# sephiroce/srf

Measured on AMD Instinct MI355X. Metric: acoustic frames/sec through SRF (123-d fbank, 3-iter DR) at 1/2/4/8 MI355X, higher is better.
Workload: dtype fp32; 1 GPU; wsj_c4: SRF L=6 PH=CH=16 DIM=32 LPAD=RPAD=2 DR iter=3, train step (fwd+bwd+allreduce+Adam); utterances_per_gpu=28, frames_per_utterance=800, global_batch=28, parallelism=dp1, launch=hipgraph (fwd+CTC+bwd)

## Files before the change

### srf_amd/csrc/route_dr.hip

```cpp
#include <algorithm>
#include <cmath>
#include <type_traits>

#include "srf_common.h"
#include "route_fwd32.h"
#include "../../include/srf.h"
#include "../../include/srf_prof.h"

namespace {

constexpr float kSquashEps = 1e-7f;

thread_local hipEvent_t* t_ev_start = nullptr;
thread_local hipEvent_t* t_ev_stop = nullptr;
thread_local int t_ev_n = 0;
constexpr int MODE_FWD = 0;
constexpr int MODE_BWD = 1;

using srf::DrGeom;

template <int KS>
__device__ __forceinline__ void load_vec(const float* __restrict__ p, float (&v)[KS]) {
  if constexpr (KS % 4 == 0) {
#pragma unroll
// ... 557 lines not shown
  const int lane = threadIdx.x & 63, wv = threadIdx.x >> 6;
  const int fl = lane & 15, g = lane >> 4;
  const int chunk = blockIdx.x % n_chunks;
  const int rest = blockIdx.x / n_chunks;
  const int wgrp = rest % n_wgroups;
  const int ft = rest / n_wgroups;
  const int f = ft * 16 + fl;
  const FrameLoc loc = frame_loc(f, F, T);
  const int tbase = __builtin_amdgcn_readfirstlane((wgrp * NW + wv) * TW);
  const int n0 = chunk * n_per, nn = min(N, n0 + n_per) - n0;
  const int Wn = in_n / N;
  const int ncap = Wn * nn;
  const int Jeff = J - (mask_first ? 1 : 0);
  const int SROW = gu_row_stride(n_per, DIN);
  const int nslots = 15 + Wn;
  float* gw_acc = gacc + (size_t)wv * nslots_max * SROW;
  for (int k = threadIdx.x; k < NW * nslots_max * SROW; k += blockDim.x) gacc[k] = 0.f;
  __syncthreads();

  float vcr[RV][TW][4], gsr[R][TW][4];
  float c0[TW];
#pragma unroll
  for (int t = 0; t < TW; ++t) {
    const int j = tile_j<DIN>(tbase + t, g);
    c0[t] = (j < J && !(mask_first && j == 0)) ? 1.f / (float)Jeff : 0.f;
#pragma unroll
    for (int r = 0; r < R; ++r) {
      if (r > 0) load_rows(saved + (size_t)(2 * (r - 1) + 1) * FJD, f, loc.valid, JD, tbase + t, g, vcr[r - 1][t]);
      load_rows(gs + (size_t)r * FJD, f, loc.valid, JD, tbase + t, g, gsr[r][t]);
    }
  }
  const int Fs = srf::fwd32_frame_stride(F);
  const uint32_t cblk_b = (uint32_t)in_n * JP * Fs * 4;
  const auto rs_w = __builtin_amdgcn_make_buffer_rsrc(const_cast<float*>(WT), 0, (int)((size_t)in_n * NT * 16 * DIN * 4),
                                                       0x00020000);
  const auto rs_c = __builtin_amdgcn_make_buffer_rsrc(const_cast<float*>(cst), 0, (int)(cblk_b * RV), 0x00020000);
  const auto rs_g = __builtin_amdgcn_make_buffer_rsrc(const_cast<float*>(glst), 0, (int)(cblk_b * RV), 0x00020000);
  uint32_t wo[NCT][TW], co[TW];
#pragma unroll
  for (int t = 0; t < TW; ++t) {
    const int tc = min(tbase + t, NT - 1);
#pragma unroll
    for (int ct = 0; ct < NCT; ++ct)
      wo[ct][t] = (uint32_t)(((tc * 4 + g) * DIN + min(ct * 16 + fl, DIN - 1)) * 4) * 4;
    co[t] = (uint32_t)(min(tile_j<DIN>(tbase + t, g), J - 1) * Fs + (loc.valid ? f : 0)) * 4;
  }
  constexpr int NB = 3;
  f4 wt_b[NB][NCT][TW];
  float c_b[NB][RV][TW], g_b[NB][RV][TW];
  auto fetch = [&](auto slot, int i) {
    constexpr int sl = decltype(slot)::value;
    const uint32_t sw = (uint32_t)i * NT * 16 * DIN * 4;
    const uint32_t sc = (uint32_t)i * JP * Fs * 4;
#pragma unroll
    for (int ct = 0; ct < NCT; ++ct)
#pragma unroll
      for (int t = 0; t < TW; ++t)
        wt_b[sl][ct][t] = __builtin_bit_cast(f4, __builtin_amdgcn_raw_buffer_load_b128(rs_w, wo[ct][t], sw, 0));
#pragma unroll
    for (int r = 0; r < RV; ++r)
#pragma unroll
      for (int t = 0; t < TW; ++t) {
        c_b[sl][r][t] = __builtin_bit_cast(float, __builtin_amdgcn_raw_buffer_load_b32(rs_c, co[t], sc + r * cblk_b, 0));
        g_b[sl][r][t] = __builtin_bit_cast(float, __builtin_amdgcn_raw_buffer_load_b32(rs_g, co[t], sc + r * cblk_b, 0));
      }
  };
  int w = 0, nl = 0, wf = 0, nf = 0;
  auto advance = [&](int& ww, int& nn_) {
    if (++nn_ == nn) nn_ = 0, ++ww;
  };
  auto compute = [&](auto slot) {
    constexpr int sl = decltype(slot)::value;
    const int i = w * N + n0 + nl;
    float ga[TW][4];
#pragma unroll
    for (int t = 0; t < TW; ++t)
#pragma unroll
      for (int h = 0; h < 2; ++h) {
        f2 a = c0[t] * f2{gsr[0][t][2 * h], gsr[0][t][2 * h + 1]};
#pragma unroll
        for (int r = 0; r < RV; ++r) {
          a = c_b[sl][r][t] * f2{gsr[r + 1][t][2 * h], gsr[r + 1][t][2 * h + 1]} + a;
          a = g_b[sl][r][t] * f2{vcr[r][t][2 * h], vcr[r][t][2 * h + 1]} + a;
        }
        ga[t][2 * h] = a.x;
        ga[t][2 * h + 1] = a.y;
      }
    f4 gx[NCT];
#pragma unroll
    for (int ct = 0; ct < NCT; ++ct) {
      gx[ct] = f4{0.f, 0.f, 0.f, 0.f};
#pragma unroll
      for (int t = 0; t < TW; ++t)
#pragma unroll
        for (int q = 0; q < 4; ++q) gx[ct] = mfma16x16x4(wt_b[sl][ct][t][q], ga[t][q], gx[ct]);
    }
    const int ts = loc.t + w - lpad;
    if (loc.valid && ts >= 0 && ts < T) {
      const int n = i - w * N;
#pragma unroll
      for (int ct = 0; ct < NCT; ++ct) {
        if (ct * 16 + 4 * g >= DIN) continue;
        float* a = gw_acc + (fl + w) * SROW + gu_acc_col<DIN>(fl + w, (n - n0) * DIN + ct * 16 + 4 * g);
        st4(a, ld4(a) + gx[ct]);
      }
    }
    advance(w, nl);
  };
  using S0 = std::integral_constant<int, 0>;
  using S1 = std::integral_constant<int, 1>;
  using S2 = std::integral_constant<int, 2>;
  const int i_last = (Wn - 1) * N + n0 + nn - 1;
  auto next_i = [&]() {
    const int i = min(wf * N + n0 + nf, i_last);
    advance(wf, nf);
    return i;
  };
#define SRF_GUX_FETCH(SL) \
  fetch(SL{}, next_i());  \
  __builtin_amdgcn_sched_barrier(0);
  if (ncap > 0) {
    SRF_GUX_FETCH(S0)
    SRF_GUX_FETCH(S1)
  }
  for (int k = 0; k < ncap; k += NB) {
    SRF_GUX_FETCH(S2)
    compute(S0{});
    if (k + 1 >= ncap) break;
    SRF_GUX_FETCH(S0)
    compute(S1{});
    if (k + 2 >= ncap) break;
    SRF_GUX_FETCH(S1)
    compute(S2{});
  }
#undef SRF_GUX_FETCH
  __syncthreads();
  const int f0 = ft * 16 - lpad;
  const int row = nn * DIN;
  for (int k = threadIdx.x; k < nslots * row; k += blockDim.x) {
    const int slot = k / row, rem = k - slot * row;
    const int fo = f0 + slot;
    float v = 0.f;
    const int pos = gu_acc_col<DIN>(slot, rem);
    for (int q = 0; q < NW; ++q) v += gacc[((size_t)q * nslots_max + slot) * SROW + pos];
    if (fo >= 0 && fo < F && v != 0.f) atomicAdd(g_emb + ((size_t)fo * N + n0) * DIN + rem, v);
  }
}

#ifndef SRF_GUX16_XCD
#define SRF_GUX16_XCD 1
#endif
#ifndef SRF_GW16S_XCD
#define SRF_GW16S_XCD 1
#endif
typedef _Float16 h8 __attribute__((ext_vector_type(8)));
typedef float f16v __attribute__((ext_vector_type(16)));
typedef _Float16 h2 __attribute__((ext_vector_type(2)));
constexpr int kGux16NW = 4;
constexpr int kGux16Occ = 2;

__device__ __forceinline__ f16v mfma32h(const h8& a, const h8& b, const f16v& c) {
  return __builtin_amdgcn_mfma_f32_32x32x16_f16(a, b, c, 0, 0, 0);
}

__device__ __forceinline__ void split8h(const f2 (&a)[4], h8& hi, h8& lo) {
#pragma unroll
  for (int v = 0; v < 4; ++v) {
    const f2 hf = __builtin_bit_cast(f2, __builtin_bit_cast(u2, a[v]) & 0xFFFFE000u);
    const h2 ph = __builtin_convertvector(hf, h2), pl = __builtin_convertvector(a[v] - hf, h2);
    hi[2 * v] = ph[0];
    hi[2 * v + 1] = ph[1];
    lo[2 * v] = pl[0];
    lo[2 * v + 1] = pl[1];
  }
}

template <int R>
__global__ __launch_bounds__(64 * kGux16NW, kGux16Occ) void route_gux16_kernel(
    const float* __restrict__ WT, const float* __restrict__ hdr, int F, int T, int N, int lpad, int in_n, int J,
    int mask_first, int n_wgroups, int n_chunks, int n_per, const float* __restrict__ saved,
    const float* __restrict__ gs, float* __restrict__ g_emb, const float* __restrict__ cst,
    const float* __restrict__ glst, int JP, float* __restrict__ gumax, int jgpw) {
  static_assert(R >= 2, "stored couplings exist for iters >= 2");
  constexpr int DIN = 32, RV = R - 1, NW = kGux16NW;
  extern __shared__ __attribute__((aligned(16))) float gacc[];
  const int JD = J * DIN;
  const int NT = JD / 16;
  const size_t FJD = (size_t)F * JD;
  const int lane = threadIdx.x & 63, wv = threadIdx.x >> 6;
  const int fl = lane & 31, h = lane >> 5;
#if SRF_GUX16_XCD
  const int n_ft = (F + 31) / 32, n_tasks = n_ft * n_wgroups * n_chunks;
  const int task = (int)(blockIdx.x & 7) * (int)(gridDim.x >> 3) + (int)(blockIdx.x >> 3);
  if (task >= n_tasks) return;
  const int chunk = task % n_chunks;
  const int rest = task / n_chunks;
  const int ft = rest % n_ft;
  const int wgrp = rest / n_ft;
#else
  const int chunk = blockIdx.x % n_chunks;
  const int rest = blockIdx.x / n_chunks;
  const int wgrp = rest % n_wgroups;
  const int ft = rest / n_wgroups;
#endif
  const int f = ft * 32 + fl;
  const FrameLoc loc = frame_loc(f, F, T);
  const int fv = loc.valid ? f : 0;
  const int n0 = chunk * n_per, nn = min(N, n0 + n_per) - n0;
  const int Wn = in_n / N;
  const int ncap = Wn * nn;
  const int Jeff = J - (mask_first ? 1 : 0);
  const int SROW = n_per * DIN + 4;
  const int nslots = 31 + Wn;
  float* slab = gacc + (size_t)wv * nslots * SROW;
  for (int k = threadIdx.x; k < NW * nslots * SROW / 4; k += blockDim.x) st4(gacc + 4 * k, f4{0.f, 0.f, 0.f, 0.f});
  __syncthreads();
  float gmax = 0.f;
  for (int jg = 0; jg < jgpw; ++jg) {
  const int jw = (wgrp * jgpw + jg) * NW + wv;
  const bool wave_on = jw < J;
  const int j = __builtin_amdgcn_readfirstlane(min(jw, J - 1));

  const float c0 = (wave_on && !(mask_first && j == 0)) ? 1.f / (float)Jeff : 0.f;
  float gsr[R][16], vcr[RV][16];
  {
    const bool ok = loc.valid && wave_on;
    auto rows = [&](const float* base, float (&o)[16]) {
      const float* p = base + (size_t)fv * JD + j * DIN + 8 * h;
#pragma unroll
      for (int ks = 0; ks < 2; ++ks)
#pragma unroll
        for (int q = 0; q < 2; ++q) {
          const f4 a = ld4(p + 16 * ks + 4 * q);
          o[8 * ks + 4 * q] = ok ? a.x : 0.f;
          o[8 * ks + 4 * q + 1] = ok ? a.y : 0.f;
          o[8 * ks + 4 * q + 2] = ok ? a.z : 0.f;
          o[8 * ks + 4 * q + 3] = ok ? a.w : 0.f;
        }
    };
#pragma unroll
    for (int r = 0; r < R; ++r) {
      rows(gs + (size_t)r * FJD, gsr[r]);
      if (r > 0) rows(saved + (size_t)(2 * (r - 1) + 1) * FJD, vcr[r - 1]);
    }
  }
  float gm[R], vm[RV];
  {
    auto rowmax = [&](const float (&o)[16]) {
      float m = 0.f;
#pragma unroll
      for (int k = 0; k < 16; k += 2) m = fmaxf(m, fmaxf(fabsf(o[k]), fabsf(o[k + 1])));
      float ma, mb;
      xpair32(m, ma, mb);
      return fmaxf(ma, mb);
    };
#pragma unroll
    for (int r = 0; r < R; ++r) {
      gm[r] = rowmax(gsr[r]);
      if (r > 0) vm[r - 1] = rowmax(vcr[r - 1]);
    }
    gm[0] *= c0;
  }
  const int aw = (int)hdr[1];
  const int Fs = srf::fwd32_frame_stride(F);
  const uint32_t cblk_b = (uint32_t)in_n * JP * Fs * 4;
  const uint32_t wplane = (uint32_t)in_n * NT * 16 * DIN * 2;
  const auto rs_w = __builtin_amdgcn_make_buffer_rsrc(const_cast<float*>(WT), 0, (int)(2 * wplane), 0x00020000);
  const auto rs_c = __builtin_amdgcn_make_buffer_rsrc(const_cast<float*>(cst), 0, (int)(cblk_b * RV), 0x00020000);
  const auto rs_g = __builtin_amdgcn_make_buffer_rsrc(const_cast<float*>(glst), 0, (int)(cblk_b * RV), 0x00020000);
  uint32_t wo[2][2];
#pragma unroll
  for (int ks = 0; ks < 2; ++ks)
#pragma unroll
    for (int p = 0; p < 2; ++p) wo[ks][p] = (uint32_t)((((2 * j + ks) * 2 + h) * DIN + fl) * 16) + p * wplane;
  const uint32_t co = (uint32_t)(j * Fs + fv) * 4;
  constexpr int NB = 3;
  h8 wt_b[NB][2][2];
  float c_b[NB][RV], g_b[NB][RV];
  auto fetch = [&](auto slot, int i) {
    constexpr int sl = decltype(slot)::value;
    const uint32_t swo = (uint32_t)i * NT * 16 * DIN * 2;
    const uint32_t sc = (uint32_t)i * JP * Fs * 4;
#pragma unroll
    for (int ks = 0; ks < 2; ++ks)
#pragma unroll
      for (int p = 0; p < 2; ++p)
        wt_b[sl][ks][p] = __builtin_bit_cast(h8, __builtin_amdgcn_raw_buffer_load_b128(rs_w, wo[ks][p], swo, 0));
#pragma unroll
    for (int r = 0; r < RV; ++r) {
      c_b[sl][r] = __builtin_bit_cast(float, __builtin_amdgcn_raw_buffer_load_b32(rs_c, co, sc + r * cblk_b, 0));
      g_b[sl][r] = __builtin_bit_cast(float, __builtin_amdgcn_raw_buffer_load_b32(rs_g, co, sc + r * cblk_b, 0));
    }
  };
  int w = 0, nl = 0, wf = 0, nf = 0;
  auto advance = [&](int& ww, int& nn_) {
    if (++nn_ == nn) nn_ = 0, ++ww;
  };
  auto compute = [&](auto slot) {
    constexpr int sl = decltype(slot)::value;
    float mh = gm[0];
#pragma unroll
    for (int r = 0; r < RV; ++r) mh = fmaf(fabsf(g_b[sl][r]), vm[r], fmaf(fabsf(c_b[sl][r]), gm[r + 1], mh));
    gmax = fmaxf(gmax, mh);
    const int eg = srf_split_exp(mh);
    const float sg = srf_exp2i(eg);
    const float s0 = c0 * sg;
// ... 382 lines not shown
  constexpr int SF = CAP * PC;
  constexpr int SFL = CAP * PCL;
  constexpr int NQ = (SF / 4 + 255) / 256;
  __shared__ __attribute__((aligned(16))) float stg[2][SFL];
  const int JD = J * D;
  const int NT = (JD + 15) / 16;
  const size_t FJD = (size_t)F * JD;
  const int Fs = srf::fwd32_frame_stride(F);
  const size_t cblk = (size_t)in_n * JP * Fs;
  const int lane = threadIdx.x & 63, wv = threadIdx.x >> 6;
  const int l16 = lane & 15, kk = lane >> 4;
  int L = blockIdx.x;
  const int s = L % S;
  L /= S;
  const int rtg = L % n_rt;
  const int cc = L / n_rt;
  const int tg = rtg * 4 + wv;
  const int row = min(tg * 16 + l16, JD - 1);
  const bool rvalid = tg < NT && tg * 16 + l16 < JD;
  const int j = row / D;
  const int jg0 = (rtg * 64) / D;
  const int jl = min(j - jg0, JW - 1);
  const int Jeff = J - (mask_first ? 1 : 0);
  const float c0 = (rvalid && j < J && !(mask_first && j == 0)) ? 1.f / (float)Jeff : 0.f;
  const int i0 = cc * CAP, ncap = min(in_n, i0 + CAP) - i0;
  const int NFT = Fp >> 4;
  const int ft0 = s * ft_per, ft1 = min(NFT, ft0 + ft_per);

  const float* src[NQ];
  int dst[NQ];
#pragma unroll
  for (int q = 0; q < NQ; ++q) {
    const int idx = min(q * 256 + (int)threadIdx.x, SF / 4 - 1);
    const int k = idx / (PC / 4), rem = idx - k * (PC / 4);
    const int i = i0 + min(k, ncap - 1);
    if (rem < CG / 4) {
      const int fq = rem & 3, jw = (rem >> 2) % JW, cg = (rem >> 2) / JW;
      const int jj = min(jg0 + jw, JP - 1);
      src[q] = ((cg & 1) ? glst : cst) + (size_t)(cg >> 1) * cblk + ((size_t)i * JP + jj) * Fs + 4 * fq;
      dst[q] = k * PCL + rem * 4;
    } else {
      const int x = rem - CG / 4;
      src[q] = xT + ((size_t)i * D + (x >> 2)) * Fp + 4 * (x & 3);
      const int e = x >> 2;
      dst[q] = k * PCL + CG + e * 16 + 4 * ((x & 3) ^ ((e >> 1) & 3));
    }
  }
  f4 sv[NQ];
  auto stage_load = [&](int ft) {
#pragma unroll
    for (int q = 0; q < NQ; ++q) sv[q] = ld4(src[q] + ft * 16);
  };
  auto stage_store = [&](int buf) {
#pragma unroll
    for (int q = 0; q < NQ; ++q) {
      const int idx = q * 256 + threadIdx.x;
      if ((SF / 4) % 256 == 0 || idx < SF / 4) st4(&stg[buf][dst[q]], sv[q]);
    }
  };
  const uint32_t nrec = (uint32_t)(FJD * 4);
  __amdgpu_buffer_rsrc_t rs_g[R], rs_v[RV];
#pragma unroll
  for (int r = 0; r < R; ++r) {
    rs_g[r] = __builtin_amdgcn_make_buffer_rsrc(const_cast<float*>(gs + (size_t)r * FJD), 0, (int)nrec, 0x00020000);
    if (r > 0)
      rs_v[r - 1] = __builtin_amdgcn_make_buffer_rsrc(const_cast<float*>(saved + (size_t)(2 * (r - 1) + 1) * FJD), 0,
                                                      (int)nrec, 0x00020000);
  }
  const uint32_t vo0 = (uint32_t)((4 * kk) * JD + row) * 4;
  float g0[4], gr[RV][4], vr[RV][4];
  float n0[4], nr[RV][4], nvr[RV][4];
  auto vec_load = [&](int ft) {
#pragma unroll
    for (int v = 0; v < 4; ++v) {
      const uint32_t o = vo0 + (uint32_t)((ft * 16 + v) * JD) * 4;
      n0[v] = __builtin_bit_cast(float, __builtin_amdgcn_raw_buffer_load_b32(rs_g[0], o, 0, 0));
#pragma unroll
      for (int r = 0; r < RV; ++r) {
        nr[r][v] = __builtin_bit_cast(float, __builtin_amdgcn_raw_buffer_load_b32(rs_g[r + 1], o, 0, 0));
        nvr[r][v] = __builtin_bit_cast(float, __builtin_amdgcn_raw_buffer_load_b32(rs_v[r], o, 0, 0));
      }
    }
  };

  f4 acc[CAP][NCT];
  float gb[CAP];
#pragma unroll
  for (int k = 0; k < CAP; ++k) {
    gb[k] = 0.f;
#pragma unroll
    for (int ct = 0; ct < NCT; ++ct) acc[k][ct] = f4{0.f, 0.f, 0.f, 0.f};
  }
  if (ft0 < ft1) {
    stage_load(ft0);
    vec_load(ft0);
    stage_store(0);
    if (ft0 + 1 < ft1) stage_load(ft0 + 1);
  }
  for (int ft = ft0; ft < ft1; ++ft) {
    const int buf = (ft - ft0) & 1;
#pragma unroll
    for (int v = 0; v < 4; ++v) {
      g0[v] = n0[v];
#pragma unroll
      for (int r = 0; r < RV; ++r) gr[r][v] = nr[r][v], vr[r][v] = nvr[r][v];
    }
    __syncthreads();
    if (ft + 1 < ft1) {
      stage_store(buf ^ 1);
      if (ft + 2 < ft1) stage_load(ft + 2);
    }
    vec_load(ft + 1 < ft1 ? ft + 1 : ft);
    const float* sb = stg[buf];
#pragma unroll
    for (int k = 0; k < CAP; ++k) {
      const float* ck = sb + k * PCL;
      float gu[4];
#pragma unroll
      for (int v = 0; v < 4; ++v) gu[v] = c0 * g0[v];
#pragma unroll
      for (int r = 0; r < RV; ++r) {
        const f4 c = ld4(ck + ((r * 2 + 0) * JW + jl) * 16 + 4 * kk);
        const f4 gl = ld4(ck + ((r * 2 + 1) * JW + jl) * 16 + 4 * kk);
#pragma unroll
        for (int v = 0; v < 4; ++v) gu[v] += c[v] * gr[r][v] + gl[v] * vr[r][v];
      }
      gb[k] += (gu[0] + gu[1]) + (gu[2] + gu[3]);
#pragma unroll
      for (int ct = 0; ct < NCT; ++ct) {
        const int e = min(ct * 16 + l16, D - 1);
        const f4 xa = ld4(ck + CG + e * 16 + 4 * (kk ^ ((e >> 1) & 3)));
#pragma unroll
        for (int v = 0; v < 4; ++v) acc[k][ct] = mfma16x16x4(xa[v], gu[v], acc[k][ct]);
      }
    }
  }
  float* gw = gwp + (size_t)s * pstride;
  float* gbo = gbp + (size_t)s * pstride;
#pragma unroll
  for (int k = 0; k < CAP; ++k) {
    if (k >= ncap) continue;
    const int i = i0 + k;
    const float t = xor32_sum(xor16_sum(gb[k]));
    if (rvalid) {
      if (kk == 0) gbo[(size_t)i * JD + row] = t;
#pragma unroll
      for (int ct = 0; ct < NCT; ++ct)
        if (ct * 16 + 4 * kk < D) st4(gw + ((size_t)i * JD + row) * D + ct * 16 + 4 * kk, acc[k][ct]);
    }
  }
}

constexpr int kGw16Cap = 4;
template <int R, int CAP>
__global__ __launch_bounds__(256, 2) void route_gw16s_kernel(
    const _Float16* __restrict__ x16, const float* __restrict__ hdr, const float* __restrict__ gumax,
    const float* __restrict__ saved, const float* __restrict__ gs, const float* __restrict__ cst,
    const float* __restrict__ glst, int F, int Fp, int in_n, int J, int mask_first, int JP, int n_rt, int S,
    int ft_per, float* __restrict__ gwp, float* __restrict__ gbp, size_t pstride) {
  static_assert(R >= 2 && R <= 3, "stored couplings exist for iters >= 2; registers hold R <= 3");
  constexpr int D = 32, RV = R - 1;
  constexpr int CG = RV * 2 * 4 * 16;
  constexpr int PQ = CG / 4 + 128;
  constexpr int PCB = CG * 4 + 2 * D * 16 * 2;
  constexpr int NQ = (CAP * PQ + 255) / 256;
  __shared__ __attribute__((aligned(16))) unsigned char stg[2][CAP * PCB];
  const int JD = J * D;
  const size_t FJD = (size_t)F * JD;
  const int Fs = srf::fwd32_frame_stride(F);
  const size_t cblk = (size_t)in_n * JP * Fs;
  const int lane = threadIdx.x & 63, wv = threadIdx.x >> 6;
  const int n = lane & 31, h = lane >> 5;
#if SRF_GW16S_XCD
  const int n_cc = (in_n + CAP - 1) / CAP, n_tasks = n_cc * n_rt * S;
  const int task = (int)(blockIdx.x & 7) * (int)(gridDim.x >> 3) + (int)(blockIdx.x >> 3);
  if (task >= n_tasks) return;
  const int cc = task % n_cc;
  const int rtg = (task / n_cc) % n_rt;
  const int s = task / n_cc / n_rt;
#else
  int b = blockIdx.x;
  const int s = b % S;
  b /= S;
  const int rtg = b % n_rt;
  const int cc = b / n_rt;
#endif
  const int jw = rtg * 4 + wv;
  const bool wave_on = jw < J;
  const int j = min(jw, J - 1);
  const int row = j * D + n;
  const int Jeff = J - (mask_first ? 1 : 0);
  const float c0 = (wave_on && !(mask_first && j == 0)) ? 1.f / (float)Jeff : 0.f;
  const int i0 = cc * CAP, ncap = min(in_n, i0 + CAP) - i0;
  const int NFT = Fp >> 4;
  const int ft0 = s * ft_per, ft1 = min(NFT, ft0 + ft_per);
  const int bx = (int)hdr[2];
  const int eg = srf_split_exp(*gumax);
  const float sg = srf_exp2i(eg);

  constexpr int NCPL = CAP * CG / 4;
  const char* src[NQ];
  int dst[NQ];
  bool cpl[NQ];
#pragma unroll
  for (int q = 0; q < NQ; ++q) {
    const int idx = min(q * 256 + (int)threadIdx.x, CAP * PQ - 1);
    cpl[q] = (q + 1) * 256 <= NCPL || (q * 256 < NCPL && idx < NCPL);
    if (cpl[q]) {
      const int k = idx / (CG / 4), rem = idx - k * (CG / 4);
      const int i = i0 + min(k, ncap - 1);
      const int fq = rem & 3, jq = (rem >> 2) & 3, cg = rem >> 4;
      const int jj = min(rtg * 4 + jq, JP - 1);
      src[q] = reinterpret_cast<const char*>(((cg & 1) ? glst : cst) + (size_t)(cg >> 1) * cblk +
                                             ((size_t)i * JP + jj) * Fs + 4 * fq);
      dst[q] = k * PCB + rem * 16;
    } else {
      const int x = idx - NCPL, k = x >> 7, xr = x & 127;
      const int p = xr >> 6, e = (xr >> 1) & 31, hf = xr & 1;
      const int i = i0 + min(k, ncap - 1);
      src[q] = reinterpret_cast<const char*>(x16 + (((size_t)i * NFT * 2 + p) * 32 + e) * 16 + hf * 8);
      dst[q] = k * PCB + CG * 4 + p * (D * 16 * 2) + (e * 16 + ((hf ^ ((e >> 3) & 1)) * 8)) * 2;
    }
  }
  f4 sv[NQ];
  auto stage_load = [&](int ft) {
#pragma unroll
    for (int q = 0; q < NQ; ++q) sv[q] = *reinterpret_cast<const f4*>(src[q] + (size_t)ft * (cpl[q] ? 64 : 2 * 32 * 16 * 2));
  };
  auto stage_store = [&](int buf) {
#pragma unroll
    for (int q = 0; q < NQ; ++q) {
      const int idx = q * 256 + threadIdx.x;
      if ((CAP * PQ) % 256 != 0 && idx >= CAP * PQ) continue;
      *reinterpret_cast<f4*>(&stg[buf][dst[q]]) = cpl[q] ? sv[q] * sg : sv[q];
    }
  };
  const uint32_t nrec = (uint32_t)(FJD * 4);
  __amdgpu_buffer_rsrc_t rs_g[R], rs_v[RV];
#pragma unroll
  for (int r = 0; r < R; ++r) {
    rs_g[r] = __builtin_amdgcn_make_buffer_rsrc(const_cast<float*>(gs + (size_t)r * FJD), 0, (int)nrec, 0x00020000);
    if (r > 0)
      rs_v[r - 1] = __builtin_amdgcn_make_buffer_rsrc(const_cast<float*>(saved + (size_t)(2 * (r - 1) + 1) * FJD), 0,
                                                      (int)nrec, 0x00020000);
  }
  const uint32_t vo0 = (uint32_t)((8 * h) * JD + row) * 4;
  f2 nxa[R + RV][4], nxb[R + RV][4];
  auto vec_load = [&](f2 (&nx)[R + RV][4], int ft) {
#pragma unroll
    for (int v = 0; v < 8; ++v) {
      const uint32_t so = (uint32_t)((ft * 16 + v) * JD) * 4;
#pragma unroll
      for (int r = 0; r < R; ++r) {
        nx[r][v >> 1][v & 1] = __builtin_bit_cast(float, __builtin_amdgcn_raw_buffer_load_b32(rs_g[r], vo0, so, 0));
        if (r > 0) nx[R + r - 1][v >> 1][v & 1] = __builtin_bit_cast(float, __builtin_amdgcn_raw_buffer_load_b32(rs_v[r - 1], vo0, so, 0));
      }
    }
  };

  f16v acc[CAP];
  float gb[CAP];
#pragma unroll
  for (int k = 0; k < CAP; ++k) {
    gb[k] = 0.f;
    acc[k] = f16v{};
  }
  if (ft0 < ft1) {
    stage_load(ft0);
    vec_load(nxa, ft0);
    stage_store(0);
    if (ft0 + 1 < ft1) stage_load(ft0 + 1);
  }
  const int xoff = CG * 4 + (n * 16 + ((h ^ ((n >> 3) & 1)) * 8)) * 2;
  const float s0 = c0 * sg;
  auto tile = [&](auto bufc, const f2 (&cur)[R + RV][4], f2 (&nxt)[R + RV][4], int ft) {
    constexpr int buf = decltype(bufc)::value;
    f2 g0[4];
#pragma unroll
    for (int v = 0; v < 4; ++v) g0[v] = cur[0][v] * s0;
    __syncthreads();
    if (ft + 1 < ft1) {
      stage_store(buf ^ 1);
      if (ft + 2 < ft1) stage_load(ft + 2);
    }
    vec_load(nxt, ft + 1 < ft1 ? ft + 1 : ft);
    const unsigned char* sb = stg[buf];
#pragma unroll
    for (int k = 0; k < CAP; ++k) {
      const unsigned char* ck = sb + k * PCB;
      const float* ckf = reinterpret_cast<const float*>(ck);
      f2 gu[4];
#pragma unroll
      for (int v = 0; v < 4; ++v) gu[v] = g0[v];
#pragma unroll
      for (int r = 0; r < RV; ++r) {
        const float* cp = ckf + ((r * 2 + 0) * 4 + wv) * 16 + 8 * h;
        const float* gp = ckf + ((r * 2 + 1) * 4 + wv) * 16 + 8 * h;
        const f4 ca = ld4(cp), cb = ld4(cp + 4), ga = ld4(gp), gbv = ld4(gp + 4);
        const f2 c2[4] = {f2{ca[0], ca[1]}, f2{ca[2], ca[3]}, f2{cb[0], cb[1]}, f2{cb[2], cb[3]}};
        const f2 g2[4] = {f2{ga[0], ga[1]}, f2{ga[2], ga[3]}, f2{gbv[0], gbv[1]}, f2{gbv[2], gbv[3]}};
#pragma unroll
        for (int v = 0; v < 4; ++v) {
          gu[v] = __builtin_elementwise_fma(c2[v], cur[r + 1][v], gu[v]);
          gu[v] = __builtin_elementwise_fma(g2[v], cur[R + r][v], gu[v]);
        }
      }
      const f2 gq = (gu[0] + gu[1]) + (gu[2] + gu[3]);
      gb[k] += gq[0] + gq[1];
      h8 bh, bl;
      split8h(gu, bh, bl);
      const h8 xh = *reinterpret_cast<const h8*>(ck + xoff);
      const h8 xl = *reinterpret_cast<const h8*>(ck + xoff + D * 16 * 2);
      acc[k] = mfma32h(xh, bh, acc[k]);
      acc[k] = mfma32h(xh, bl, acc[k]);
      acc[k] = mfma32h(xl, bh, acc[k]);
    }
  };
  using S0 = std::integral_constant<int, 0>;
  using S1 = std::integral_constant<int, 1>;
  for (int ft = ft0; ft < ft1; ft += 2) {
    tile(S0{}, nxa, nxb, ft);
    if (ft + 1 >= ft1) break;
    tile(S1{}, nxb, nxa, ft + 1);
  }
  float* gw = gwp + (size_t)s * pstride;
  float* gbo = gbp + (size_t)s * pstride;
  const float un = srf_exp2i(-(bx + eg)), ug = srf_exp2i(-eg);
#pragma unroll
  for (int k = 0; k < CAP; ++k) {
    const float a = gb[k];
    float pa, pb;
    xpair32(a, pa, pb);
    if (k >= ncap || !wave_on) continue;
    const int i = i0 + k;
    if (h == 0) gbo[(size_t)i * JD + row] = (pa + pb) * ug;
#pragma unroll
    for (int q = 0; q < 4; ++q)
      st4(gw + ((size_t)i * JD + row) * D + 8 * q + 4 * h,
          f4{acc[k][4 * q] * un, acc[k][4 * q + 1] * un, acc[k][4 * q + 2] * un, acc[k][4 * q + 3] * un});
  }
}

__global__ void gw_reduce_kernel(const float* __restrict__ part, int S, size_t n4, size_t stride, float* __restrict__ gW,
                                 size_t nw4, float* __restrict__ gb) {
  const size_t idx = (size_t)blockIdx.x * blockDim.x + threadIdx.x;
  if (idx >= n4) return;
  f4 a = ld4(part + idx * 4);
  for (int s = 1; s < S; ++s) a += ld4(part + (size_t)s * stride + idx * 4);
  if (idx < nw4)
    st4(gW + idx * 4, a);
  else
    st4(gb + (idx - nw4) * 4, a);
}

template <int Q>
__device__ __forceinline__ float qsum(float v) {
#pragma unroll
  for (int o = 1; o < Q; o <<= 1) v += __shfl_xor(v, o, 64);
  return v;
}

struct SlabSplit {
  int n;
  int G, U, in_n, JD;
};

__device__ __forceinline__ int slab_count(const SlabSplit& sp, size_t FJD, size_t off) {
  if (sp.G <= 0) return sp.n;
  const uint32_t f = FJD <= 0xffffffffu ? (uint32_t)off / (uint32_t)sp.JD : (uint32_t)(off / (size_t)sp.JD);
  return srf::bal_tile_slots((int)(f >> 5), sp.in_n, sp.U, sp.G);
}

__device__ __forceinline__ f4 sum_slab4(const float* __restrict__ slab, const SlabSplit& sp, size_t FJD, size_t off) {
  const int n = slab_count(sp, FJD, off);
  f4 a = ld4(slab + off);
#pragma unroll 4
  for (int c = 1; c < n; ++c) a += ld4(slab + (size_t)c * FJD + off);
  return a;
}

template <int DOUT>
__global__ void fwd_finish_kernel(const float* __restrict__ slab, SlabSplit sp, size_t FJD,
                                  const float* __restrict__ vc_in, float* __restrict__ s_out,
                                  float* __restrict__ vc_out, float* __restrict__ v_out) {
  constexpr int Q = DOUT / 4;
  const size_t idx = (size_t)blockIdx.x * blockDim.x + threadIdx.x;
  const bool ok = idx < FJD / 4;
  const size_t off = (ok ? idx : 0) * 4;
  const f4 sv = sum_slab4(slab, sp, FJD, off);
  const float n2 = qsum<Q>((sv.x * sv.x + sv.y * sv.y) + (sv.z * sv.z + sv.w * sv.w));
  if (!ok) return;
  const float fac = n2 / (1.f + n2) / sqrtf(n2 + kSquashEps);
  const f4 v = sv * fac;
  st4(s_out + off, sv);
  if (vc_out) st4(vc_out + off, vc_in ? v + ld4(vc_in + off) : v);
  if (v_out) st4(v_out + off, v);
}

template <int DOUT>
__global__ void bwd_finish_kernel(const float* __restrict__ slab, SlabSplit sp, size_t FJD,
                                  const float* __restrict__ a_init, float* __restrict__ A,
                                  const float* __restrict__ s, float* __restrict__ gs, float* __restrict__ zero4,
                                  size_t nz4, float* __restrict__ zero1) {
  constexpr int Q = DOUT / 4;
  const size_t idx = (size_t)blockIdx.x * blockDim.x + threadIdx.x;
  if (idx < nz4) st4(zero4 + idx * 4, f4{0.f, 0.f, 0.f, 0.f});
  if (zero1 != nullptr && idx == 0) *zero1 = 0.f;
  const bool ok = idx < FJD / 4;
  const size_t off = (ok ? idx : 0) * 4;
  f4 a;
  if (a_init) {
    a = ld4(a_init + off);
    if (ok) st4(A + off, f4{0.f, 0.f, 0.f, 0.f});
  } else {
    a = ld4(A + off) + sum_slab4(slab, sp, FJD, off);
    if (ok) st4(A + off, a);
  }
  const f4 sv = ld4(s + off);
  const float n2 = qsum<Q>((sv.x * sv.x + sv.y * sv.y) + (sv.z * sv.z + sv.w * sv.w));
  const float sa = qsum<Q>((sv.x * a.x + sv.y * a.y) + (sv.z * a.z + sv.w * a.w));
  if (!ok) return;
  const float rs = 1.f / sqrtf(n2 + kSquashEps);
  const float ip = 1.f / (1.f + n2);
  const float gfac = n2 * ip * rs;
  const float dg2 = 2.f * rs * ip * (ip - 0.5f * n2 / (n2 + kSquashEps)) * sa;
  st4(gs + off, a * gfac + sv * dg2);
}

struct PassCfg {
  int TW, NW;
};

PassCfg pass_cfg(const DrGeom& g) {
  const int NT = g.NT();
  int TW = 8;
  int NW = (NT + TW - 1) / TW;
  if (NW > 8) {
    TW = 16;
    NW = (NT + TW - 1) / TW;
  }
  return {TW, NW};
}

int auto_chunks(const DrGeom& g, int NW) {
  const int n_ftiles = (g.F() + 15) / 16;
  const int wg_per_cu = std::max(1, 8 / NW);
  const int slots = 256 * wg_per_cu;
  int best = 1;
  double best_cost = 1e30;
  for (int c = 1; c <= std::min(g.in_n(), 96); ++c) {
    const int rounds = (n_ftiles * c + slots - 1) / slots;
    const int len = (g.in_n() + c - 1) / c;
    double cost = (double)rounds * (len + 2);
    if (8 % c != 0 && c % 8 != 0) cost *= 1.05;
    cost *= 1.0 + 0.002 * c;
    if (cost < best_cost) {
      best_cost = cost;
      best = c;
    }
  }
  return best;
}

template <int D, int TW, int MODE>
void launch_pass(const DrGeom& g, int NW, int n_chunks, const float* emb, const float* W, const float* bias, int r,
                 const float* vc, const float* gsv, float* slab, float* stats, int want_acc, hipStream_t st) {
  const int n_ftiles = (g.F() + 15) / 16;
  const int chunk_len = (g.in_n() + n_chunks - 1) / n_chunks;
  const size_t shmem = (NW > 1) ? (size_t)2 * NW * 48 * sizeof(float) : 16;
  auto kern = r == 0 ? route_pass_kernel<D, D, TW, MODE, true> : route_pass_kernel<D, D, TW, MODE, false>;
  hipLaunchKernelGGL(kern, dim3(n_ftiles * n_chunks), dim3(64 * NW), shmem, st,
                     emb, W, bias, g.F(), g.T, g.N, g.lpad, g.in_n(), g.J, n_chunks, chunk_len, g.mask_first, r,
                     vc, gsv, slab, stats, want_acc);
}

template <int D, int MODE>
void dispatch_pass(const DrGeom& g, const PassCfg& pc, int n_chunks, const float* emb, const float* W,
                   const float* bias, int r, const float* vc, const float* gsv, float* slab, float* stats,
                   int want_acc, hipStream_t st) {
  if (pc.TW == 8)
    launch_pass<D, 8, MODE>(g, pc.NW, n_chunks, emb, W, bias, r, vc, gsv, slab, stats, want_acc, st);
  else
    launch_pass<D, 16, MODE>(g, pc.NW, n_chunks, emb, W, bias, r, vc, gsv, slab, stats, want_acc, st);
}

template <int D>
void launch_fwd_finish(const DrGeom& g, const float* slab, const SlabSplit& sp, const float* vc_in, float* s_out,
// ... 46 lines not shown
inline size_t gux16_lds_bytes(const DrGeom& g, int n_per) {
  return (size_t)kGux16NW * (31 + gu_window(g)) * (n_per * 32 + 4) * sizeof(float);
}
constexpr size_t kGux16LdsMax = (160 / kGux16Occ - 4) * 1024;
int gux16_n_per(const DrGeom& g, int jgpw) {
  const int base = (g.F() + 31) / 32 * ((g.J + kGux16NW - 1) / kGux16NW / jgpw);
  const int slots = 256 * kGux16Occ;
  int best = 1;
  double best_cost = 1e30;
  for (int n_per = 1; n_per <= g.N; ++n_per) {
    if (n_per > 1 && gux16_lds_bytes(g, n_per) > kGux16LdsMax) break;
    const int chunks = (g.N + n_per - 1) / n_per;
    const int rounds = (base * chunks + slots - 1) / slots;
    const double cost = (double)rounds * (gu_window(g) * n_per * jgpw + 4);
    if (cost < best_cost) {
      best_cost = cost;
      best = n_per;
    }
  }
  return best;
}

struct Gw2Plan {
  int cap, n_rt, n_cc, S, ft_per;
  size_t pstride;
};
constexpr int gw3_capsules(int d) { return d <= 16 ? 8 : 4; }

enum class GxPass {
  kRecompute,
  kStored,
  kStored16,
};
enum class GwPass {
  kFromGu,
  kGw2,
  kGw3,
  kGw16s,
};

struct BwdWs {
  size_t A, gs, slab, stats, gu_t, xT, WT;
  size_t gumax;
  size_t p32;
  size_t gl;
  size_t gwpart;
  size_t bytes;
};

struct DrPlan {
  DrGeom g;
  bool fwd32;
  srf::Fwd32Plan p32;
  srf::Fwd32Cpl cpl;
  Gw2Plan gw2;
  bool can_store;
  bool couplings;
  PassCfg pc;
  int chunks;
  int plan_arg;
  GxPass gx;
  GwPass gw;
  size_t fwd_bytes;
  BwdWs ws;
  int JP() const { return p32.JDp / g.dout; }
  const float* hdr(const float* cpl_base) const { return srf::fwd32_hdr(p32, cpl_base + cpl.planes); }
};

#ifndef SRF_GUX16_JGPW
#define SRF_GUX16_JGPW 2
#endif
template <int R>
void launch_gux16(const DrGeom& g, const float* WT, const float* hdr, const float* saved, const float* gs,
                  float* g_emb, const float* cst, const float* glst, int JP, float* gumax, hipStream_t st) {
  const int n_all = (g.J + kGux16NW - 1) / kGux16NW;
  const int jgpw = n_all % SRF_GUX16_JGPW == 0 ? SRF_GUX16_JGPW : 1;
  const int n_wgroups = n_all / jgpw;
  const int n_per = gux16_n_per(g, jgpw);
  const int n_chunks = (g.N + n_per - 1) / n_per;
  int grid = (g.F() + 31) / 32 * n_wgroups * n_chunks;
  if (SRF_GUX16_XCD) grid = (grid + 7) / 8 * 8;
  hipLaunchKernelGGL((route_gux16_kernel<R>), dim3(grid), dim3(64 * kGux16NW), gux16_lds_bytes(g, n_per), st, WT, hdr,
                     g.F(), g.T, g.N, g.lpad, g.in_n(), g.J, g.mask_first, n_wgroups, n_chunks, n_per, saved, gs, g_emb,
                     cst, glst, JP, gumax, jgpw);
}

template <int D, int R>
void launch_gu(const DrPlan& p, const float* emb, const float* W, const float* WT, const float* bias,
               const float* saved, const float* gs, const float* stats, float* gu_t, float* g_emb, hipStream_t st,
               const float* cst, const float* glst, const float* hdr, float* gumax) {
  const DrGeom& g = p.g;
  if constexpr (D == 32 && R >= 2 && R <= 4) {
    if (p.gx == GxPass::kStored16) {
      launch_gux16<R>(g, WT, hdr, saved, gs, g_emb, cst, glst, p.JP(), gumax, st);
      return;
    }
  }
  const int n_ftiles = (g.F() + 15) / 16;
  const int n_wgroups = gu_wgroups(g);
  constexpr int TW = gu_tw(D);
  const int nw = std::min(kGuNW, (g.NT() + TW - 1) / TW);
  const int n_per = gu_n_per(g, nw);
  const int n_chunks = (g.N + n_per - 1) / n_per;
  const int nslots = 15 + gu_window(g);
  const size_t lds = gu_lds_bytes(g, nw, n_per);
  if constexpr (R >= 2 && D <= 32) {
    if (p.gx == GxPass::kStored) {
      hipLaunchKernelGGL((route_gux_kernel<D, TW, R>), dim3(n_ftiles * n_wgroups * n_chunks), dim3(64 * nw), lds, st,
                         WT, g.F(), g.T, g.N, g.lpad, g.in_n(), g.J, g.mask_first, n_wgroups, n_chunks, n_per, saved,
                         gs, g_emb, nslots, cst, glst, p.JP());
      return;
    }
  }
  const bool ldsacc = lds <= kGuLdsMax;
  hipLaunchKernelGGL((ldsacc ? route_gu_kernel<D, D, TW, R, true> : route_gu_kernel<D, D, TW, R, false>),
                     dim3(n_ftiles * n_wgroups * n_chunks), dim3(64 * nw), ldsacc ? lds : 0, st, emb, W, WT, bias, g.F(),
                     padded_frames(g), g.T, g.N, g.lpad, g.rpad, g.in_n(), g.J, g.mask_first, n_wgroups, n_chunks, n_per,
                     saved, gs, stats, gu_t, g_emb, nslots, nullptr, nullptr, 0);
}

template <int V>
using Int = std::integral_constant<int, V>;

template <class Fn>
auto dispatch_iters(int iters, Fn&& fn) {
  switch (iters) {
    case 1: return fn(Int<1>{});
    case 2: return fn(Int<2>{});
    case 3: return fn(Int<3>{});
    case 4: return fn(Int<4>{});
    default: return fn(Int<5>{});
  }
}
template <class Fn>
int dispatch_din(int din, Fn&& fn) {
  switch (din) {
    case 8: return fn(Int<8>{});
    case 16: return fn(Int<16>{});
    case 32: return fn(Int<32>{});
    default: return fn(Int<64>{});
  }
}

template <int D>
int launch_gw2(const DrPlan& pl, const float* xT, const float* saved, const float* gs, const float* cst,
               const float* glst, float* gwp, float* gbp, hipStream_t st, const float* hdr, const float* gumax) {
  static_assert(D <= 32, "couplings are stored by the 32x32 forward");
  const DrGeom& g = pl.g;
  const Gw2Plan& p = pl.gw2;
  const int JP = pl.JP(), Fp = padded_frames(g);
  const int grid = p.n_rt * p.n_cc * p.S;
  if constexpr (D == 32) {
    if (pl.gw == GwPass::kGw16s) {
      const int grid16 = SRF_GW16S_XCD ? (grid + 7) / 8 * 8 : grid;
      const _Float16* x16 = reinterpret_cast<const _Float16*>(xT);
      hipLaunchKernelGGL((g.iters == 2 ? route_gw16s_kernel<2, kGw16Cap> : route_gw16s_kernel<3, kGw16Cap>), dim3(grid16),
                         dim3(256), 0, st, x16, hdr, gumax, saved, gs, cst, glst, g.F(), Fp, g.in_n(), g.J, g.mask_first,
                         JP, p.n_rt, p.S, p.ft_per, gwp, gbp, p.pstride);
      SRF_LAUNCH_CHECK("route_gw16s");
      return SRF_OK;
    }
  }
  if (pl.gw == GwPass::kGw3) {
    constexpr int CAP = gw3_capsules(D);
    hipLaunchKernelGGL((g.iters == 2 ? route_gw3_kernel<D, 2, CAP> : route_gw3_kernel<D, 3, CAP>), dim3(grid), dim3(256),
                       0, st, xT, saved, gs, cst, glst, g.F(), Fp, g.in_n(), g.J, g.mask_first, JP, p.n_rt, p.S, p.ft_per,
                       gwp, gbp, p.pstride);
    SRF_LAUNCH_CHECK("route_gw3");
    return SRF_OK;
  }
  hipLaunchKernelGGL((g.iters == 4 ? route_gw2_kernel<D, 4> : route_gw2_kernel<D, 5>), dim3(grid), dim3(256), 0, st, xT,
                     saved, gs, cst, glst, g.F(), Fp, g.in_n(), g.J, g.mask_first, JP, p.n_rt, p.n_cc, p.S, p.ft_per, gwp,
                     gbp, p.pstride);
  SRF_LAUNCH_CHECK("route_gw2");
  return SRF_OK;
}


inline bool use_fwd32(const DrGeom& g) { return srf::fwd32_supported(g.din, g.dout, g.J); }

inline bool use_gux16(const DrGeom& g) {
  return g.din == 32 && g.dout == 32 && g.iters >= 2 && g.iters <= 4 &&
         gux16_lds_bytes(g, 1) <= kGux16LdsMax;
}
inline bool use_gw16s(const DrGeom& g) { return use_gux16(g) && g.iters <= 3; }

inline int gw3_cap(const DrGeom& g) { return g.iters <= 3 && g.din <= 32 ? gw3_capsules(g.din) : 0; }

Gw2Plan gw2_plan(const DrGeom& g, GwPass kind) {
  const bool g16 = kind == GwPass::kGw16s, g3 = kind == GwPass::kGw3;
  Gw2Plan p{};
  const int NT = g.NT();
  const int NCT = g16 ? 2 : (g.din + 15) / 16;
  p.n_rt = g16 ? (g.J + 3) / 4 : (NT + 3) / 4;
  p.cap = g16 ? kGw16Cap : g3 ? gw3_capsules(g.din) : (g.din <= 16 ? 8 : 4);
  const int slots = g16 ? 512 : g3 ? 2 * 768 : 512;
  const double per_tile = g16 ? 120.0 : 200.0;
  p.n_cc = (g.in_n() + p.cap - 1) / p.cap;
  const int NFT = padded_frames(g) / 16;
  p.pstride = (size_t)g.in_n() * g.JD() * (g.din + 1);
  const int base = p.n_rt * p.n_cc;
  double best = 1e30;
  for (int S0 = 1; S0 <= NFT; ++S0) {
    const int ft_per = (NFT + S0 - 1) / S0;
    const int S = (NFT + ft_per - 1) / ft_per;
    const int rounds = (base * S + slots - 1) / slots;
    const double work = (double)rounds * ft_per * p.cap * NCT * per_tile / 2.4e9;
    const double slab = S > 1 ? 2.0 * S * p.pstride * 4 / 4e12 : 0.0;
    if (work + slab < best) {
      best = work + slab;
      p.S = S;
      p.ft_per = ft_per;
    }
  }
  return p;
}

inline bool couplings_ok(const DrGeom& g, const srf::Fwd32Cpl& cpl) {
  if (!use_fwd32(g) || g.iters < 2 || g.din > 32) return false;
  constexpr size_t kLim = size_t(1) << 31;
  const int TW = gu_tw(g.dout);
  const int nw = std::min(kGuNW, (g.NT() + TW - 1) / TW);
  return gu_lds_bytes(g, nw, 1) <= kGuLdsMax && cpl.total * 4 < kLim && (size_t)g.F() * g.JD() * 4 * g.iters < kLim;
}

inline bool plan_balanced(int n_chunks) { return n_chunks > 0 && (n_chunks & srf::kBalFlag) != 0; }
inline bool plan_arg_ok(const DrPlan& p, int n_chunks) {
  return plan_balanced(n_chunks) ? p.fwd32 : (n_chunks >= 1 && n_chunks <= p.g.in_n());
}

void resolve(DrPlan& p, const DrGeom& g, int n_chunks, bool have_couplings) {
  p = DrPlan{};
  p.g = g;
  p.fwd32 = use_fwd32(g);
  p.pc = pass_cfg(g);
  p.chunks = plan_balanced(n_chunks) ? auto_chunks(g, p.pc.NW) : n_chunks;
  p.fwd_bytes = plan_balanced(n_chunks) ? 0 : (size_t)n_chunks * ((size_t)g.B * g.T + 1) * g.J * g.dout * sizeof(float);
  GwPass stored_gw = GwPass::kGw2;
  if (p.fwd32) {
    p.p32 = srf::fwd32_plan(g, n_chunks);
    p.fwd_bytes = std::max(p.fwd_bytes, srf::fwd32_workspace(p.p32));
    p.cpl = srf::fwd32_cpl_layout(p.p32, g);
    stored_gw = use_gw16s(g) ? GwPass::kGw16s : gw3_cap(g) ? GwPass::kGw3 : GwPass::kGw2;
    p.gw2 = gw2_plan(g, stored_gw);
  }
  p.plan_arg = p.fwd32 ? p.p32.plan_arg : n_chunks == 0 ? auto_chunks(g, p.pc.NW) : p.chunks;
  p.can_store = couplings_ok(g, p.cpl);
  p.couplings = have_couplings && p.can_store;
  p.gx = !p.couplings ? GxPass::kRecompute : use_gux16(g) ? GxPass::kStored16 : GxPass::kStored;
  p.gw = p.couplings ? stored_gw : GwPass::kFromGu;

  const size_t F = g.F(), JD = g.JD(), in_n = g.in_n(), Fp = padded_frames(g);
  size_t off = 0;
  auto take = [&](size_t nfloat) {
    const size_t o = off;
    off += srf::align_up(nfloat * sizeof(float), 256);
    return o / sizeof(float);
  };
  BwdWs& w = p.ws;
  w.A = take(F * JD);
  w.gs = take((size_t)g.iters * F * JD);
  w.slab = take((size_t)p.chunks * F * JD);
  w.stats = take((size_t)(g.iters - 1) * F * in_n * 2);
  w.gu_t = take(in_n * (size_t)g.NT() * 16 * Fp);
  w.xT = take(in_n * g.din * Fp);
  w.WT = take(in_n * JD * g.din);
  w.gumax = take(64);
  if (p.fwd32) {
    w.p32 = take((srf::fwd32_scratch_bytes(p.p32) + 3) / 4);
    w.gl = take((size_t)std::max(g.iters - 1, 1) * srf::fwd32_frame_stride(g.F()) * in_n * p.JP());
    w.gwpart = take((size_t)p.gw2.S * p.gw2.pstride);
  }
  w.bytes = off;
}

int check_geom(const DrGeom& g) {
  SRF_REQUIRE(g.B > 0 && g.T > 0 && g.N > 0 && g.J > 1, "bad shape B=%d T=%d N=%d J=%d", g.B, g.T, g.N, g.J);
  SRF_REQUIRE(g.lpad >= 0 && g.rpad >= 0, "negative window pad");
  SRF_REQUIRE(g.iters >= 1 && g.iters <= 5, "routing iterations must be in [1,5], got %d", g.iters);
  SRF_REQUIRE(g.din == 8 || g.din == 16 || g.din == 32 || g.din == 64, "unsupported in_d %d", g.din);
  SRF_REQUIRE(g.dout == g.din, "in_d (%d) != out_d (%d) is not supported", g.din, g.dout);
  SRF_REQUIRE((long long)g.F() * g.in_n() * g.JD() < (1LL << 40), "problem too large");
  return SRF_OK;
}

inline SlabSplit uniform_split(int n) { return SlabSplit{n, 0, 0, 0, 0}; }
inline SlabSplit pass_split(const DrGeom& g, const srf::Fwd32Plan& p) {
  return p.bal_G > 0 ? SlabSplit{p.n_slots, p.bal_G, p.bal_U, g.in_n(), g.JD()} : uniform_split(p.n_chunks);
}

template <int D>
int fwd_impl(const DrPlan& p, const float* emb, const float* W, const float* bias, float* v_out, float* saved,
             float* couplings, float* slab, hipStream_t st) {
  const DrGeom& g = p.g;
  const srf::Fwd32Plan& plan = p.p32;
  const srf::Fwd32Cpl& cl = p.cpl;
  const size_t FJD = (size_t)g.F() * g.JD();
  hipEvent_t* ev0 = t_ev_start;
  hipEvent_t* ev1 = t_ev_stop;
  const int nev = t_ev_n;
  t_ev_start = t_ev_stop = nullptr;
  t_ev_n = 0;
  float* bsum = nullptr;
  void* planes = slab;
  void* scratch = slab;
  if (p.fwd32) {
    float *WT = nullptr, *xT = nullptr;
    if (p.couplings) {
      planes = couplings + cl.planes;
      WT = couplings + cl.WT;
      xT = couplings + cl.xT;
// ... 328 lines not shown
```

Before: 2.958 million frames/s.

## Share per-frame vector tiles across two capsule groups via LDS image in gw16s

The gw16s weight-gradient kernel now runs 512-thread blocks in which two 256-thread groups handle different capsule sets but share the same routing vector tiles. Each lane issues one 128-bit buffer load per vector stream instead of eight scalar loads, writes into a swizzled, double-buffered LDS image, and reads its fragment back from LDS. This halves redundant global loads of gs/saved and widens the access pattern, in exchange for extra LDS traffic and capacity, larger blocks, and halving the grid.

```diff
diff --git a/srf_amd/csrc/route_dr.hip b/srf_amd/csrc/route_dr.hip
--- a/srf_amd/csrc/route_dr.hip
+++ b/srf_amd/csrc/route_dr.hip
@@ -733,6 +733,9 @@
 #endif
 #ifndef SRF_GW16S_XCD
 #define SRF_GW16S_XCD 1
+#endif
+#ifndef SRF_GW16S_LDSVEC
+#define SRF_GW16S_LDSVEC 2
 #endif
 typedef _Float16 h8 __attribute__((ext_vector_type(8)));
 typedef float f16v __attribute__((ext_vector_type(16)));
@@ -1421,27 +1424,32 @@
 }
 
 constexpr int kGw16Cap = 4;
-template <int R, int CAP>
-__global__ __launch_bounds__(256, 2) void route_gw16s_kernel(
+template <int R, int CAP, int VW>
+__global__ __launch_bounds__(VW == 2 ? 512 : 256, 2) void route_gw16s_kernel(
     const _Float16* __restrict__ x16, const float* __restrict__ hdr, const float* __restrict__ gumax,
     const float* __restrict__ saved, const float* __restrict__ gs, const float* __restrict__ cst,
     const float* __restrict__ glst, int F, int Fp, int in_n, int J, int mask_first, int JP, int n_rt, int S,
     int ft_per, float* __restrict__ gwp, float* __restrict__ gbp, size_t pstride) {
   static_assert(R >= 2 && R <= 3, "stored couplings exist for iters >= 2; registers hold R <= 3");
-  constexpr int D = 32, RV = R - 1;
+  static_assert(VW == 0 || VW == 2, "0: per-lane loads, 2: image shared by two waves");
+  constexpr int D = 32, RV = R - 1, NV = R + RV;
+  constexpr int NG = VW == 2 ? 2 : 1;
+  constexpr int NT = 256 * NG, CAPW = CAP * NG;
   constexpr int CG = RV * 2 * 4 * 16;
   constexpr int PQ = CG / 4 + 128;
   constexpr int PCB = CG * 4 + 2 * D * 16 * 2;
-  constexpr int NQ = (CAP * PQ + 255) / 256;
-  __shared__ __attribute__((aligned(16))) unsigned char stg[2][CAP * PCB];
+  constexpr int NQ = (CAPW * PQ + NT - 1) / NT;
+  constexpr int IMG = NV * D * 16;
+  __shared__ __attribute__((aligned(16))) unsigned char stg[2][CAPW * PCB];
+  __shared__ __attribute__((aligned(16))) float vimg[VW == 0 ? 4 : 2 * 4 * IMG];
   const int JD = J * D;
   const size_t FJD = (size_t)F * JD;
   const int Fs = srf::fwd32_frame_stride(F);
   const size_t cblk = (size_t)in_n * JP * Fs;
-  const int lane = threadIdx.x & 63, wv = threadIdx.x >> 6;
+  const int lane = threadIdx.x & 63, wv = (threadIdx.x >> 6) & 3, wg = threadIdx.x >> 8;
   const int n = lane & 31, h = lane >> 5;
 #if SRF_GW16S_XCD
-  const int n_cc = (in_n + CAP - 1) / CAP, n_tasks = n_cc * n_rt * S;
+  const int n_cc = (in_n + CAPW - 1) / CAPW, n_tasks = n_cc * n_rt * S;
   const int task = (int)(blockIdx.x & 7) * (int)(gridDim.x >> 3) + (int)(blockIdx.x >> 3);
   if (task >= n_tasks) return;
   const int cc = task % n_cc;
@@ -1460,21 +1468,21 @@
   const int row = j * D + n;
   const int Jeff = J - (mask_first ? 1 : 0);
   const float c0 = (wave_on && !(mask_first && j == 0)) ? 1.f / (float)Jeff : 0.f;
-  const int i0 = cc * CAP, ncap = min(in_n, i0 + CAP) - i0;
+  const int i0 = cc * CAPW, ncap = min(in_n, i0 + CAPW) - i0, k0 = wg * CAP;
   const int NFT = Fp >> 4;
   const int ft0 = s * ft_per, ft1 = min(NFT, ft0 + ft_per);
   const int bx = (int)hdr[2];
   const int eg = srf_split_exp(*gumax);
   const float sg = srf_exp2i(eg);
 
-  constexpr int NCPL = CAP * CG / 4;
+  constexpr int NCPL = CAPW * CG / 4;
   const char* src[NQ];
   int dst[NQ];
   bool cpl[NQ];
 #pragma unroll
   for (int q = 0; q < NQ; ++q) {
-    const int idx = min(q * 256 + (int)threadIdx.x, CAP * PQ - 1);
-    cpl[q] = (q + 1) * 256 <= NCPL || (q * 256 < NCPL && idx < NCPL);
+    const int idx = min(q * NT + (int)threadIdx.x, CAPW * PQ - 1);
+    cpl[q] = (q + 1) * NT <= NCPL || (q * NT < NCPL && idx < NCPL);
     if (cpl[q]) {
       const int k = idx / (CG / 4), rem = idx - k * (CG / 4);
       const int i = i0 + min(k, ncap - 1);
@@ -1499,8 +1507,8 @@
   auto stage_store = [&](int buf) {
 #pragma unroll
     for (int q = 0; q < NQ; ++q) {
-      const int idx = q * 256 + threadIdx.x;
-      if ((CAP * PQ) % 256 != 0 && idx >= CAP * PQ) continue;
+      const int idx = q * NT + threadIdx.x;
+      if ((CAPW * PQ) % NT != 0 && idx >= CAPW * PQ) continue;
       *reinterpret_cast<f4*>(&stg[buf][dst[q]]) = cpl[q] ? sv[q] * sg : sv[q];
     }
   };
@@ -1514,8 +1522,8 @@
                                                       (int)nrec, 0x00020000);
   }
   const uint32_t vo0 = (uint32_t)((8 * h) * JD + row) * 4;
-  f2 nxa[R + RV][4], nxb[R + RV][4];
-  auto vec_load = [&](f2 (&nx)[R + RV][4], int ft) {
+  f2 nxa[NV][4], nxb[NV][4];
+  auto vec_load = [&](f2 (&nx)[NV][4], int ft) {
 #pragma unroll
     for (int v = 0; v < 8; ++v) {
       const uint32_t so = (uint32_t)((ft * 16 + v) * JD) * 4;
@@ -1526,6 +1534,30 @@
       }
     }
   };
+  const int rq = lane & 7, fm = lane >> 3;
+  const uint32_t wo0 = (uint32_t)((8 * wg + fm) * JD + j * D + 4 * rq) * 4;
+  f4 vst[NV];
+  auto img_load = [&](int ft) {
+    const uint32_t so = (uint32_t)(ft * 16 * JD) * 4;
+#pragma unroll
+    for (int r = 0; r < R; ++r) {
+      vst[r] = __builtin_bit_cast(f4, __builtin_amdgcn_raw_buffer_load_b128(rs_g[r], wo0, so, 0));
+      if (r > 0) vst[R + r - 1] = __builtin_bit_cast(f4, __builtin_amdgcn_raw_buffer_load_b128(rs_v[r - 1], wo0, so, 0));
+    }
+  };
+  const int iwo = 4 * rq * 16 + 4 * ((2 * wg + (fm >> 2)) ^ (rq & 3)) + (fm & 3);
+  const int iro = n * 16 + 4 * ((2 * h) ^ ((n >> 2) & 3));
+  auto img_store = [&](float* im, int v) {
+#pragma unroll
+    for (int c = 0; c < 4; ++c) im[v * (D * 16) + iwo + c * 16] = vst[v][c];
+  };
+  auto img_read = [&](const float* im, f2 (&nx)[NV][4]) {
+#pragma unroll
+    for (int v = 0; v < NV; ++v) {
+      const f4 a = ld4(im + v * (D * 16) + iro), b = ld4(im + v * (D * 16) + (iro ^ 4));
+      nx[v][0] = f2{a[0], a[1]}, nx[v][1] = f2{a[2], a[3]}, nx[v][2] = f2{b[0], b[1]}, nx[v][3] = f2{b[2], b[3]};
+    }
+  };
 
   f16v acc[CAP];
   float gb[CAP];
@@ -1534,26 +1566,23 @@
     gb[k] = 0.f;
     acc[k] = f16v{};
   }
+  float* const imw = vimg + wv * IMG;
   if (ft0 < ft1) {
     stage_load(ft0);
-    vec_load(nxa, ft0);
+    if constexpr (VW == 0) vec_load(nxa, ft0);
+    else img_load(ft0);
     stage_store(0);
     if (ft0 + 1 < ft1) stage_load(ft0 + 1);
+    if constexpr (VW == 2) {
+#pragma unroll
+      for (int v = 0; v < NV; ++v) img_store(imw, v);
+      img_load(min(ft0 + 1, ft1 - 1));
+    }
   }
   const int xoff = CG * 4 + (n * 16 + ((h ^ ((n >> 3) & 1)) * 8)) * 2;
   const float s0 = c0 * sg;
-  auto tile = [&](auto bufc, const f2 (&cur)[R + RV][4], f2 (&nxt)[R + RV][4], int ft) {
-    constexpr int buf = decltype(bufc)::value;
-    f2 g0[4];
-#pragma unroll
-    for (int v = 0; v < 4; ++v) g0[v] = cur[0][v] * s0;
-    __syncthreads();
-    if (ft + 1 < ft1) {
-      stage_store(buf ^ 1);
-      if (ft + 2 < ft1) stage_load(ft + 2);
-    }
-    vec_load(nxt, ft + 1 < ft1 ? ft + 1 : ft);
-    const unsigned char* sb = stg[buf];
+  auto caps = [&](int buf, const f2 (&g0)[4], const f2 (&cur)[NV][4], bool img_next) {
+    const unsigned char* sb = stg[buf] + k0 * PCB;
 #pragma unroll
     for (int k = 0; k < CAP; ++k) {
       const unsigned char* ck = sb + k * PCB;
@@ -1583,14 +1612,51 @@
       acc[k] = mfma32h(xh, bh, acc[k]);
       acc[k] = mfma32h(xh, bl, acc[k]);
       acc[k] = mfma32h(xl, bh, acc[k]);
-    }
+      if constexpr (VW == 2) {
+        if (img_next) {
+#pragma unroll
+          for (int v = 0; v < NV; ++v)
+            if (v * CAP / NV == k) img_store(imw + (buf ^ 1) * (4 * IMG), v);
+        }
+      }
+    }
+  };
+  auto tile = [&](auto bufc, const f2 (&cur)[NV][4], f2 (&nxt)[NV][4], int ft) {
+    constexpr int buf = decltype(bufc)::value;
+    f2 g0[4];
+#pragma unroll
+    for (int v = 0; v < 4; ++v) g0[v] = cur[0][v] * s0;
+    __syncthreads();
+    if (ft + 1 < ft1) {
+      stage_store(buf ^ 1);
+      if (ft + 2 < ft1) stage_load(ft + 2);
+    }
+    vec_load(nxt, ft + 1 < ft1 ? ft + 1 : ft);
+    caps(buf, g0, cur, false);
+  };
+  auto tile_img = [&](auto bufc, int ft) {
+    constexpr int buf = decltype(bufc)::value;
+    f2 cur[NV][4], g0[4];
+    __syncthreads();
+    img_read(imw + buf * (4 * IMG), cur);
+    if (ft + 1 < ft1) {
+      stage_store(buf ^ 1);
+      if (ft + 2 < ft1) stage_load(ft + 2);
+    }
+#pragma unroll
+    for (int v = 0; v < 4; ++v) g0[v] = cur[0][v] * s0;
+    caps(buf, g0, cur, ft + 1 < ft1);
+    __builtin_amdgcn_sched_barrier(0);
+    img_load(min(ft + 2, ft1 - 1));
   };
   using S0 = std::integral_constant<int, 0>;
   using S1 = std::integral_constant<int, 1>;
   for (int ft = ft0; ft < ft1; ft += 2) {
-    tile(S0{}, nxa, nxb, ft);
+    if constexpr (VW == 0) tile(S0{}, nxa, nxb, ft);
+    else tile_img(S0{}, ft);
     if (ft + 1 >= ft1) break;
-    tile(S1{}, nxb, nxa, ft + 1);
+    if constexpr (VW == 0) tile(S1{}, nxb, nxa, ft + 1);
+    else tile_img(S1{}, ft + 1);
   }
   float* gw = gwp + (size_t)s * pstride;
   float* gbo = gbp + (size_t)s * pstride;
@@ -1600,8 +1666,8 @@
     const float a = gb[k];
     float pa, pb;
     xpair32(a, pa, pb);
-    if (k >= ncap || !wave_on) continue;
-    const int i = i0 + k;
+    if (k0 + k >= ncap || !wave_on) continue;
+    const int i = i0 + k0 + k;
     if (h == 0) gbo[(size_t)i * JD + row] = (pa + pb) * ug;
 #pragma unroll
     for (int q = 0; q < 4; ++q)
@@ -1954,11 +2020,13 @@
   const int grid = p.n_rt * p.n_cc * p.S;
   if constexpr (D == 32) {
     if (pl.gw == GwPass::kGw16s) {
-      const int grid16 = SRF_GW16S_XCD ? (grid + 7) / 8 * 8 : grid;
+      constexpr int VW = SRF_GW16S_LDSVEC, NG = VW == 2 ? 2 : 1;
+      const int tasks = p.n_rt * ((p.n_cc + NG - 1) / NG) * p.S;
+      const int grid16 = SRF_GW16S_XCD ? (tasks + 7) / 8 * 8 : tasks;
       const _Float16* x16 = reinterpret_cast<const _Float16*>(xT);
-      hipLaunchKernelGGL((g.iters == 2 ? route_gw16s_kernel<2, kGw16Cap> : route_gw16s_kernel<3, kGw16Cap>), dim3(grid16),
-                         dim3(256), 0, st, x16, hdr, gumax, saved, gs, cst, glst, g.F(), Fp, g.in_n(), g.J, g.mask_first,
-                         JP, p.n_rt, p.S, p.ft_per, gwp, gbp, p.pstride);
+      hipLaunchKernelGGL((g.iters == 2 ? route_gw16s_kernel<2, kGw16Cap, VW> : route_gw16s_kernel<3, kGw16Cap, VW>),
+                         dim3(grid16), dim3(256 * NG), 0, st, x16, hdr, gumax, saved, gs, cst, glst, g.F(), Fp, g.in_n(),
+                         g.J, g.mask_first, JP, p.n_rt, p.S, p.ft_per, gwp, gbp, p.pstride);
       SRF_LAUNCH_CHECK("route_gw16s");
       return SRF_OK;
     }
```

Result: faster. 3.002 million frames/s (median of 6 runs) (+1.5%).
